# unixpickle/vq-voice-swap

Measured on AMD Instinct MI355X. Metric: audio clips/sec (whole node), unet64 50-step DDPM on 4s@16kHz waveforms, higher is better.
Workload: dtype fp16; 1 GPU; unet64 50-step DDPM (constrain, schedule t**2), 64 clips/GPU x 1 GPU of T=64000; global_batch=64, parallelism=clips sharded over 1 GPU(s), gather to rank 0

## Files before the change

### vq_voice_swap_amd/csrc/conv_ws.hip

```cpp
#include <atomic>
#include <cstddef>
#include <cstdio>
#include <cstdlib>
#include <mutex>
#include <set>
#include <string>
#include <type_traits>

#include "kernels.hpp"

namespace vqvs {

namespace {

typedef unsigned int u32x4 __attribute__((ext_vector_type(4)));
typedef int i32x4 __attribute__((ext_vector_type(4)));
typedef __attribute__((address_space(3))) void* lds_ptr;

template <typename T> struct WsOp;
template <> struct WsOp<half_t> {
  typedef f16x8 v8;
  static constexpr unsigned short one = 0x3C00;
#ifdef VQVS_F16_GELU6
  static constexpr int gq = GELU_POLY6;
// ... 15 lines not shown
__device__ __forceinline__ f32x16 ws_mfma(f16x8 a, f16x8 b, f32x16 c) { return __builtin_amdgcn_mfma_f32_32x32x16_f16(a, b, c, 0, 0, 0); }

#ifndef VQVS_WS_GELU_IL
#define VQVS_WS_GELU_IL 1
#endif
template <int Q, int N, bool IL>
__device__ __forceinline__ void ws_gelu_n(float (&v)[N]) {
  float w[N], p[N];
#define WS_G8(expr)                    \
  _Pragma("unroll") for (int i = 0; i < N; ++i) { expr; } \
  if (VQVS_WS_GELU_IL && IL) __builtin_amdgcn_sched_barrier(0);
  WS_G8(w[i] = v[i] * v[i])
  WS_G8(w[i] = __builtin_fminf(w[i], 16.0f))
  if constexpr (Q == GELU_POLY6) {
    WS_G8(p[i] = fmaf(2.81608722e-08f, w[i], -1.89188380e-06f))
    WS_G8(p[i] = fmaf(p[i], w[i], 5.41903041e-05f))
    WS_G8(p[i] = fmaf(p[i], w[i], -8.78980255e-04f))
    WS_G8(p[i] = fmaf(p[i], w[i], 9.11294959e-03f))
    WS_G8(p[i] = fmaf(p[i], w[i], -6.53883549e-02f))
    WS_G8(p[i] = fmaf(p[i], w[i], 3.98526915e-01f))
  } else {
    WS_G8(p[i] = fmaf(-1.301278171e-09f, w[i], 1.041951057e-07f))
    WS_G8(p[i] = fmaf(p[i], w[i], -3.657111166e-06f))
    WS_G8(p[i] = fmaf(p[i], w[i], 7.485478930e-05f))
    WS_G8(p[i] = fmaf(p[i], w[i], -1.006488756e-03f))
    WS_G8(p[i] = fmaf(p[i], w[i], 9.505392772e-03f))
    WS_G8(p[i] = fmaf(p[i], w[i], -6.588783436e-02f))
    WS_G8(p[i] = fmaf(p[i], w[i], 3.986733897e-01f))
  }
  WS_G8(p[i] = __builtin_amdgcn_fmed3f(fmaf(v[i], p[i], 0.5f), 0.0f, 1.0f))
  WS_G8(v[i] = v[i] * p[i])
#undef WS_G8
}

template <int Q>
__device__ __forceinline__ float ws_gelu(float v) {
  const float w = __builtin_fminf(v * v, 16.0f);
  float p;
  if constexpr (Q == GELU_POLY6) {
    p = fmaf(2.81608722e-08f, w, -1.89188380e-06f);
    p = fmaf(p, w, 5.41903041e-05f);
    p = fmaf(p, w, -8.78980255e-04f);
    p = fmaf(p, w, 9.11294959e-03f);
    p = fmaf(p, w, -6.53883549e-02f);
    p = fmaf(p, w, 3.98526915e-01f);
  } else {
    p = fmaf(-1.301278171e-09f, w, 1.041951057e-07f);
    p = fmaf(p, w, -3.657111166e-06f);
    p = fmaf(p, w, 7.485478930e-05f);
    p = fmaf(p, w, -1.006488756e-03f);
    p = fmaf(p, w, 9.505392772e-03f);
    p = fmaf(p, w, -6.588783436e-02f);
    p = fmaf(p, w, 3.986733897e-01f);
  }
  return v * __builtin_amdgcn_fmed3f(fmaf(v, p, 0.5f), 0.0f, 1.0f);
}

struct WsSeg {
  const void* src;
  const float2* ss;
  int Csrc;
  int clip_bytes;
  int c0;
  int nch;
  int ntaps;
  int dil;
  int rsz;
  int ss_lds;
  int ss_stride, ss_c0;
  int wbase, wstep;
  int lds_off;
};
struct WsGn {
  const float *part0, *part1;
  int ntiles0, ntiles1, C0, C1;
  int nsrc, Ctot, cpg, nclips;
  int tpc;
  double inv_count;
  const float *gamma, *beta, *film;
  int film_stride, film_off;
  unsigned* status;
  int guard;
};
struct WsArgs {
  WsGn gn;
  WsSeg seg[4];
  int nseg, nchunks;
  const void* w;
  const void* w_lo;
  int w_bytes;
  const float* bias;
  const void* skip;
  int skip_L, skip_rsz;
  void* out;
  float* stats;
  int Cout, Lout, TTO, ntx, nty, ntiles, ntiles_stat;
  int wres_bytes;
  int ss_bytes;
  int ss_ring;
  int rev;
  int zp;
};
static_assert(offsetof(WsArgs, gn) == 0, "gn_table reads WsGn through the kernarg segment pointer: it must stay the first member");
#define WS_SEGF(s, f) ((s) == 0 ? a.seg[0].f : ((s) == 1 ? a.seg[1].f : ((s) == 2 ? a.seg[2].f : a.seg[3].f)))

#ifndef VQVS_WS_PREP_EARLY
#define VQVS_WS_PREP_EARLY 1
#endif
constexpr int ws_lookahead(bool prep_early) { return prep_early ? 5 : 4; }
constexpr int WS_LOOKAHEAD = ws_lookahead(VQVS_WS_PREP_EARLY != 0);
constexpr int ws_ss_ring(long long spc, int lookahead) { return spc >= lookahead ? 2 : (spc >= 2 ? 4 : 8); }
constexpr int ws_ss_span(int spc, int lookahead) {
  int worst = 0;
  for (int o = 0; o < spc; ++o) {
    int clip = 0, pos = o;
    for (int i = 0; i < lookahead; ++i)
      if (++pos == spc) {
        pos = 0;
        ++clip;
      }
    worst = clip > worst ? clip : worst;
  }
  return worst;
}
constexpr bool ws_ss_ring_holds(int lookahead) {
  for (int spc = 1; spc <= 64; ++spc) {
    const int ring = ws_ss_ring(spc, lookahead);
    if ((ring & (ring - 1)) != 0 || ws_ss_span(spc, lookahead) >= ring) return false;
  }
  return true;
}
static_assert(ws_ss_ring_holds(ws_lookahead(true)) && ws_ss_ring_holds(ws_lookahead(false)),
              "the (scale, shift) ring is overwritten while a producer wave still reads it: ws_ss_ring vs. the load cursor's lookahead");
static_assert(ws_ss_ring(4, ws_lookahead(true)) == 4 && ws_ss_ring(4, ws_lookahead(false)) == 2, "ring at four steps per clip");

struct TileCo {
  int b, tx, ty;
};

#ifndef VQVS_WS_EXP
#define VQVS_WS_EXP 0
#endif

#ifdef VQVS_TIMING
__device__ unsigned long long g_ws_timing[32];
#define WS_TMARK(i)                                                \
  {                                                                \
    const unsigned long long _t = __builtin_amdgcn_s_memtime();    \
    tacc[i] += _t - tlast;                                         \
    tlast = _t;                                                    \
  }
#else
#define WS_TMARK(i)
#endif

template <typename T, int ROWS>
constexpr int ws_threads() { return sizeof(T) == 4 ? 1024 : ROWS * 4; }
template <typename T, int ROWS, int CT, bool RES, bool AVG, bool ZP = false>
__global__ __launch_bounds__((ws_threads<T, ROWS>())) void conv_ws_kernel(const WsArgs a) {
  constexpr bool X3 = sizeof(T) == 4;
  constexpr bool TALL = X3 && ROWS == 128;
  constexpr int WN = (CT == 128 && !TALL) ? 2 : 1;
  constexpr int MT = CT == 32 ? 1 : 2;
  constexpr int RW = 32 * MT;
  constexpr int NWT = ROWS / RW;
  constexpr int NWC = CT / (WN * 32);
  constexpr int NCW = NWT * NWC;
  constexpr int NPT = NCW * 64;
  constexpr int PR = ROWS * 4 / NPT;
  constexpr int HR = ROWS / 2;
  constexpr bool DB = CT == 32;
  constexpr int ES = (int)sizeof(T);
  constexpr bool L4 = AVG || (X3 && !TALL);
  static_assert(!(AVG && X3), "avg-pooled segments are not built for fp32 storage");
  static_assert(!X3 || (CT == 64 && ROWS == 256) || (CT == 128 && ROWS == 128), "fp32 storage: 256 x 64 or 128 x 128 tiles");
  static_assert(PR == 1 || PR == 2, "producer rows per chunk");
  static_assert(!TALL || !RES, "the 128 x 128 fp32 tile streams its weights (two planes of 3 x 128 x 64 B per chunk)");
  static_assert(!ZP || (!X3 && !RES && !AVG && ROWS == 256 && CT >= 64), "whole-clip tiles: 2-byte storage, streaming 256-row tiles of 64 / 128 channels");
  constexpr int ACT_BYTES = ROWS * 64;
  constexpr int W_BYTES = 3 * CT * 64;
  constexpr int ACT2 = (X3 ? 2 : 1) * ACT_BYTES, W2 = (X3 ? 2 : 1) * W_BYTES;
  constexpr int STAGE = ACT2 + W2;
  constexpr int OP = CT * 4 + 16;
  constexpr bool WPE = RES && WN == 2 && !X3;
  constexpr int ACT_STRIDE = RES ? ACT2 : STAGE;
  constexpr int WS_OFF = ACT2;
  constexpr int WS_STRIDE = STAGE;
  constexpr int O_OFF = RES ? 2 * ACT2 : 2 * STAGE;
  constexpr int O_BYTES = X3 ? 0 : (WPE ? NCW * 2048 : (ROWS / 2) * OP);
  constexpr int R_BYTES = NWT * CT * 8;
  constexpr int R_OFF = O_OFF + (DB ? 2 : 1) * O_BYTES;
  constexpr int C_OFF = R_OFF + (DB ? 2 : 1) * R_BYTES;
  constexpr int WRES_OFF = C_OFF + (RES ? 4096 : 0);
  const int SS_OFF = WRES_OFF + (RES ? (X3 ? 2 : 1) * a.wres_bytes : 0);
  constexpr int GQ = WsOp<T>::gq;
  typedef typename WsOp<T>::v8 V8;
  extern __shared__ __attribute__((aligned(16))) char smem[];

  const int tid = threadIdx.x;
  const int lane = tid & 63;
  const int wave = __builtin_amdgcn_readfirstlane(tid >> 6);
#ifdef VQVS_TIMING
  unsigned long long tacc[8] = {0, 0, 0, 0, 0, 0, 0, 0};
  unsigned long long tlast = __builtin_amdgcn_s_memtime();
  const unsigned long long t_sh0 = tlast, t_rt0 = __builtin_amdgcn_s_memrealtime();
#endif

  int tb, te;
  {
    const int nwg = (int)gridDim.x, w = (int)blockIdx.x;
    const int nx = nwg < 8 ? nwg : 8;
    const int k = w % nx, i = w / nx;
    const int nk = (nwg - k + nx - 1) / nx;
    const unsigned tot = (unsigned)a.ntiles;
    const unsigned s = tot * (unsigned)k / (unsigned)nx, e = tot * (unsigned)(k + 1) / (unsigned)nx;
    const unsigned len = e - s;
    tb = (int)(s + len * (unsigned)i / (unsigned)nk);
    te = (int)(s + len * (unsigned)(i + 1) / (unsigned)nk);
  }
  const int n = a.nchunks;
  const int Q = (te - tb) * n;
  if (Q <= 0) return;
  TileCo first;
  {
    const int ft = a.rev ? a.ntiles - 1 - tb : tb;
    const int rest = ft / a.nty;
    first.ty = ft - rest * a.nty;
    first.b = rest / a.ntx;
    first.tx = rest - first.b * a.ntx;
  }
  auto next_tile = [&](TileCo& t) {
    if (a.rev) {
      if (--t.ty < 0) {
        t.ty = a.nty - 1;
        if (--t.tx < 0) {
          t.tx = a.ntx - 1;
          --t.b;
        }
      }
    } else if (++t.ty == a.nty) {
      t.ty = 0;
      if (++t.tx == a.ntx) {
        t.tx = 0;
        ++t.b;
      }
    }
  };
  bool skipb = false;
  auto sync_lds = [&]() {
    asm volatile("s_waitcnt lgkmcnt(0)" ::: "memory");
    if (!(VQVS_WS_EXP & 32768) && !((VQVS_WS_EXP & 131072) && skipb)) __builtin_amdgcn_s_barrier();
    asm volatile("" ::: "memory");
  };

  if (wave >= NCW) {
    const int pt = tid - NPT;
    const int oct = pt & 3, r0 = pt >> 2;
    const int dst0 = r0 * 64 + ((oct ^ ((r0 >> 2) & 3)) << 4);
    struct Raw {
      u32x4 a0, a1;
      u32x4 b0, b1;
// ... 491 lines not shown
        __builtin_amdgcn_raw_buffer_store_b128(e, rs_o, v, 0, 0);
        __builtin_amdgcn_raw_buffer_store_b128(o, rs_o, v + a.Cout * 2, 0, 0);
      }
    };

    TileCo ct = first, nt_ = first;
    int cci = 0;
    struct SegW {
      int nch, ntaps, dil, wbase, wstep, lds_off;
    };
    auto fetchw = [&](int sg) -> SegW {
      const WsSeg& g = a.seg[sg];
      return SegW{g.nch, g.ntaps, g.dil, g.wbase, g.wstep, g.lds_off};
    };
    int dseg = 0, dch = 0;
    SegW dw = fetchw(0), dnx = fetchw(a.nseg > 1 ? 1 : 0);
    int d_woff = dw.wbase;
    auto wlds = [&](int par) { return dw.ntaps == 0 ? dch : (RES ? WRES_OFF + dw.lds_off + dch * dw.wstep : WS_OFF + par * WS_STRIDE); };
    if constexpr (RES) {
      const int nsg = a.nseg;
      for (int sg = 0; sg < nsg; ++sg) {
        const int np = (WS_SEGF(sg, nch) * WS_SEGF(sg, wstep)) >> 10;
        const int gb = WS_SEGF(sg, wbase), lb = WS_SEGF(sg, lds_off);
        for (int p = wave; p < np; p += NCW) {
          __builtin_amdgcn_raw_ptr_buffer_load_lds(rs_w, (lds_ptr)(smem + WRES_OFF + lb + p * 1024), 16, gb + p * 1024 + dma_lane, 0, 0, 0);
          if constexpr (X3)
            __builtin_amdgcn_raw_ptr_buffer_load_lds(rs_wl, (lds_ptr)(smem + WRES_OFF + a.wres_bytes + lb + p * 1024), 16, gb + p * 1024 + dma_lane, 0, 0, 0);
        }
      }
    }
    auto dma_advance = [&]() {
      if (++dch == dw.nch) {
        dch = 0;
        if (++dseg == a.nseg) {
          dseg = 0;
          next_tile(nt_);
        }
        dw = dnx;
        d_woff = dw.wbase;
        dnx = fetchw(dseg + 1 == a.nseg ? 0 : dseg + 1);
      } else {
        d_woff += dw.wstep;
      }
    };
    dma(dw.ntaps, d_woff, nt_, 0);
    int ntaps = dw.ntaps, d = dw.dil, wb = wlds(0);
    dma_advance();
    float bj[WN], bjn[WN];
#pragma unroll
    for (int nt = 0; nt < WN; ++nt) bjn[nt] = bj[nt] = a.bias[first.ty * CT + wc * (WN * 32) + nt * 32 + l31];
    int bias_ty = first.ty;
    const int last_b = (a.rev ? a.ntiles - te : te - 1) / (a.ntx * a.nty);
    auto reaches = [&](int c) { return a.rev ? (c >= last_b && c <= first.b) : (c >= first.b && c <= last_b); };
    if (a.gn.nsrc > 0)
      for (int i = 0; i < (a.ss_ring >> 1); ++i) {
        const int c = first.b + (a.rev ? -i : i);
        if (reaches(c)) gn_table(c);
      }
#ifdef VQVS_TIMING
    const unsigned long long t_su1 = __builtin_amdgcn_s_memtime();
#endif
    asm volatile("s_waitcnt lgkmcnt(0)" ::: "memory");
    __builtin_amdgcn_s_barrier();
#ifdef VQVS_TIMING
    const unsigned long long t_su2 = __builtin_amdgcn_s_memtime();
#endif
    constexpr int NKS = (WPE || ZP) ? 1 : 2;
    int aoff[3][NKS], aoff_d = -1;
    int aoff1[ZP ? 3 : 1];
    (void)aoff1;
    asm volatile("s_waitcnt vmcnt(0)" ::: "memory");
#ifdef VQVS_TIMING
    const unsigned long long t_su3 = __builtin_amdgcn_s_memtime();
#endif
    sync_all();
#ifdef VQVS_TIMING
    const unsigned long long t_su4 = __builtin_amdgcn_s_memtime();
#endif
    WS_TMARK(4)
    if (VQVS_WS_EXP & 1024) {
      for (int g = 0; g < Q; ++g) sync_all();
      return;
    }
    for (int g = 0; g < Q; ++g) {
      if (cci == 0) {
        if (gn_ahead != 0 && ct.b != gn_clip) {
          gn_clip = ct.b;
          if (reaches(ct.b + gn_ahead)) gn_table(ct.b + gn_ahead);
        }
        WS_TMARK(6)
        if ((n == 1 || (VQVS_WS_EXP & 256)) && pending) {
          store_tile(0, NIT);
          pending = false;
        }
        if (ct.ty != bias_ty) {
          bias_ty = ct.ty;
#pragma unroll
          for (int nt = 0; nt < WN; ++nt) bj[nt] = bjn[nt];
        }
        if (a.nty > 1) {
          TileCo nxt = ct;
          next_tile(nxt);
#pragma unroll
          for (int nt = 0; nt < WN; ++nt) bjn[nt] = a.bias[nxt.ty * CT + wc * (WN * 32) + nt * 32 + l31];
        }
#pragma unroll
        for (int nt = 0; nt < WN; ++nt)
#pragma unroll
          for (int r = 0; r < 16; ++r)
#pragma unroll
            for (int mt = 0; mt < MT; ++mt) acc[mt][nt][r] = bj[nt];
      }
      WS_TMARK(0)
      const int nx_ntaps = dw.ntaps, nx_dil = dw.dil, nx_wb = wlds((g + 1) & 1);
      if (g + 1 < Q) {
        dma(dw.ntaps, d_woff, nt_, (g + 1) & 1);
        dma_advance();
      }
      WS_TMARK(1)
      const char* const sb = smem + (g & 1) * ACT_STRIDE;
      float skv[MT][16];
      if constexpr (X3) {
        if (cci == n - 1 && a.skip != nullptr) {
          const int t0 = ct.tx * a.TTO;
          const int lastrow = t0 + min(a.TTO, a.Lout - t0);
          const int srows = a.skip_rsz == RESIZE_UP2 ? (lastrow + 1) >> 1 : (a.skip_rsz == RESIZE_AVG2 ? 2 * lastrow : lastrow);
          const __amdgpu_buffer_rsrc_t rs_s = __builtin_amdgcn_make_buffer_rsrc(
              const_cast<float*>(reinterpret_cast<const float*>(a.skip)) + (size_t)ct.b * a.skip_L * a.Cout, 0, srows * a.Cout * 4, 0x00020000);
          const int row0 = t0 + wt * RW + 4 * hh;
          const int ch4 = (ct.ty * CT + wc * (WN * 32) + l31) * 4;
#pragma unroll
          for (int mt = 0; mt < MT; ++mt)
#pragma unroll
            for (int r = 0; r < 16; ++r) {
              const int row = row0 + mt * 32 + (r & 3) + 8 * (r >> 2);
              if (a.skip_rsz == RESIZE_AVG2) {
                const float x0 = __builtin_bit_cast(float, __builtin_amdgcn_raw_buffer_load_b32(rs_s, (2 * row) * a.Cout * 4 + ch4, 0, 0));
                const float x1 = __builtin_bit_cast(float, __builtin_amdgcn_raw_buffer_load_b32(rs_s, (2 * row + 1) * a.Cout * 4 + ch4, 0, 0));
                skv[mt][r] = (x0 + x1) * 0.5f;
              } else {
                const int sr = a.skip_rsz == RESIZE_UP2 ? (row >> 1) : row;
                skv[mt][r] = __builtin_bit_cast(float, __builtin_amdgcn_raw_buffer_load_b32(rs_s, sr * a.Cout * 4 + ch4, 0, 0));
              }
            }
        }
      }
      {
        if (d != aoff_d) {
          aoff_d = d;
#pragma unroll
          for (int k = 0; k < 3; ++k) {
            if constexpr (ZP) {
              int row = wt * RW + l31 + (k - 1) * d, row1 = row + 32;
              row = (unsigned)row < 256u ? row : 255;
              row1 = (unsigned)row1 < 256u ? row1 : 255;
              aoff[k][0] = row * 64 + ((hh ^ ((row >> 2) & 3)) << 4);
              aoff1[k] = row1 * 64 + ((hh ^ ((row1 >> 2) & 3)) << 4);
            } else {
            const int row = wt * RW + l31 + k * d;
#pragma unroll
            for (int ks = 0; ks < NKS; ++ks) aoff[k][ks] = (row * 64 + ((hh ^ ((row >> 2) & 3)) << 4)) ^ (ks * 32);
            }
          }
        }
        int bad[WN][NKS];
#pragma unroll
        for (int nt = 0; nt < WN; ++nt)
#pragma unroll
          for (int ks = 0; ks < NKS; ++ks)
          bad[nt][ks] = ((ntaps != 0 ? wb + nt * (32 * 64) : ((RES ? C_OFF : WS_OFF + (g & 1) * WS_STRIDE) + (wc * WN + nt == wb ? 0 : 2048) - wc * (WN * 32 * 64))) + boff) ^ (ks * 32);
        auto tap = [&](int k) {
#pragma unroll
          for (int ks = 0; ks < 2; ++ks) {
            const int ao = NKS == 2 ? aoff[k][ks % NKS] : (aoff[k][0] ^ (ks * 32));
            const V8 a0 = *reinterpret_cast<const V8*>(sb + ao);
            V8 a1 = a0;
            if constexpr (ZP) a1 = *reinterpret_cast<const V8*>(sb + (aoff1[k] ^ (ks * 32)));
            else if constexpr (MT == 2) a1 = *reinterpret_cast<const V8*>(sb + ao + 32 * 64);
#pragma unroll
            for (int nt = 0; nt < WN; ++nt) {
              const V8 bf = *reinterpret_cast<const V8*>(smem + (NKS == 2 ? bad[nt][ks % NKS] : (bad[nt][0] ^ (ks * 32))) + k * (CT * 64));
              if constexpr (X3) {
                const V8 bl = *reinterpret_cast<const V8*>(smem + bad[nt][ks % NKS] + k * (CT * 64) + (RES ? a.wres_bytes : W_BYTES));
                const V8 a0l = *reinterpret_cast<const V8*>(sb + ACT_BYTES + ao);
                const V8 a1l = *reinterpret_cast<const V8*>(sb + ACT_BYTES + ao + 32 * 64);
                acc[0][nt] = ws_mfma(a0, bf, acc[0][nt]);
                acc[MT - 1][nt] = ws_mfma(a1, bf, acc[MT - 1][nt]);
                acc[0][nt] = ws_mfma(a0l, bf, acc[0][nt]);
                acc[MT - 1][nt] = ws_mfma(a1l, bf, acc[MT - 1][nt]);
                acc[0][nt] = ws_mfma(a0, bl, acc[0][nt]);
                acc[MT - 1][nt] = ws_mfma(a1, bl, acc[MT - 1][nt]);
              } else if (VQVS_WS_EXP & 4096) {
                asm volatile("" ::"v"(a0), "v"(a1), "v"(bf));
              } else {
                acc[0][nt] = ws_mfma(a0, bf, acc[0][nt]);
                if constexpr (MT == 2) acc[MT - 1][nt] = ws_mfma(a1, bf, acc[MT - 1][nt]);
              }
            }
          }
        };
        if (!(VQVS_WS_EXP & 16)) {
          tap(0);
          if (ntaps == 3) {
            tap(1);
            tap(2);
          }
        }
      }
      WS_TMARK(2)
      if (cci == n - 1 && (VQVS_WS_EXP & 32)) {
#pragma unroll
        for (int mt = 0; mt < MT; ++mt)
#pragma unroll
          for (int nt = 0; nt < WN; ++nt) asm volatile("" ::"v"(acc[mt][nt][0]), "v"(acc[mt][nt][15]));
        pt_ = ct;
        pbuf = obuf;
        pending = true;
      }
      if (cci == n - 1 && !(VQVS_WS_EXP & 32)) {
        int zl = 0;
        asm volatile("" : "+v"(zl));
        const int t0 = ct.tx * a.TTO;
        const int nvalid = min(a.TTO, a.Lout - t0);
        const int lim = nvalid - (wt * RW + 4 * hh) + zl;
        if (wt * RW + RW > nvalid) {
#pragma unroll
          for (int mt = 0; mt < MT; ++mt)
#pragma unroll
            for (int nt = 0; nt < WN; ++nt)
#pragma unroll
              for (int r = 0; r < 16; ++r)
                if (mt * 32 + (r & 3) + 8 * (r >> 2) >= lim) acc[mt][nt][r] = 0.f;
        }
        if constexpr (X3) {
          const int ch = ct.ty * CT + wc * (WN * 32) + l31 + zl;
          float* const outf = reinterpret_cast<float*>(a.out);
          const __amdgpu_buffer_rsrc_t rs_o = __builtin_amdgcn_make_buffer_rsrc(
              outf + (size_t)ct.b * a.Lout * a.Cout, 0, (t0 + nvalid) * a.Cout * 4, 0x00020000);
          const int row0 = t0 + wt * RW + 4 * hh;
          if (a.skip != nullptr) {
#pragma unroll
            for (int mt = 0; mt < MT; ++mt)
#pragma unroll
              for (int r = 0; r < 16; ++r) acc[mt][0][r] += skv[mt][r];
          }
          float s1 = 0.f, s2 = 0.f;
#pragma unroll
          for (int mt = 0; mt < MT; ++mt)
#pragma unroll
            for (int r = 0; r < 16; ++r) {
              const float v = acc[mt][0][r];
              s1 += v;
              s2 = fmaf(v, v, s2);
              if (!(VQVS_WS_EXP & 4))
                __builtin_amdgcn_raw_buffer_store_b32(__builtin_bit_cast(unsigned, v), rs_o, ((row0 + mt * 32 + (r & 3) + 8 * (r >> 2)) * a.Cout + ch) * 4, 0, 0);
            }
          s1 += __shfl_xor(s1, 32);
          s2 += __shfl_xor(s2, 32);
          if (hh == 0) reinterpret_cast<float2*>(smem + R_OFF)[wt * CT + wc * (WN * 32) + l31 + zl] = float2{s1, s2};
        } else if constexpr (WPE) {
          char* const priv = smem + O_OFF + wave * 2048 + zl;
          char* const wr0 = priv + (2 * hh) * 256 + l31 * 4;
          const int zlane = lane + zl;
          const int prw = zlane >> 3;
          const int rrow = (prw >> 2) * 32 + ((prw >> 1) & 1) * 4 + (prw & 1) * 2;
          const char* const rd0 = priv + prw * 256 + (zlane & 7) * 32;
          const __amdgpu_buffer_rsrc_t rs_o = __builtin_amdgcn_make_buffer_rsrc(
              outp + (size_t)ct.b * a.Lout * CT, 0, (t0 + nvalid) * (CT * 2), 0x00020000);
          const int vo0 = ((t0 + wt * 64 + rrow) * CT + wc * 64 + (zlane & 7) * 8) * 2;
          float s1[2] = {0.f, 0.f}, s2[2] = {0.f, 0.f};
#pragma unroll
          for (int j = 0; j < 4; ++j) {
#pragma unroll
            for (int mt = 0; mt < 2; ++mt)
#pragma unroll
              for (int rr = 0; rr < 2; ++rr)
#pragma unroll
                for (int nt = 0; nt < 2; ++nt) {
                  const int r = 4 * j + 2 * rr;
                  char* const o0 = wr0 + (mt * 4 + rr) * 256 + nt * 128;
                  if constexpr (WsOp<T>::one == 0x3C00) {
                    typedef _Float16 h2 __attribute__((ext_vector_type(2)));
                    const h2 ones = {(_Float16)1.0f, (_Float16)1.0f};
                    const h2 pk = {(_Float16)acc[mt][nt][r], (_Float16)acc[mt][nt][r + 1]};
                    s1[nt] = __builtin_amdgcn_fdot2(pk, ones, s1[nt], false);
                    s2[nt] = __builtin_amdgcn_fdot2(pk, pk, s2[nt], false);
                    *reinterpret_cast<h2*>(o0) = pk;
                  } else {
// ... 60 lines not shown
        }
        }
        pt_ = ct;
        pbuf = obuf;
        if constexpr (DB) obuf ^= 1;
        pending = true;
      }
      WS_TMARK(3)
      if (++cci == n) {
        cci = 0;
        next_tile(ct);
      }
      ntaps = nx_ntaps;
      d = nx_dil;
      wb = nx_wb;
      if (n > 1 && pending && cci >= 1) {
        if constexpr (!RES) asm volatile("s_waitcnt vmcnt(0)" ::: "memory");
        const int i0 = (cci - 1) * st_per, i1 = i0 + st_per;
        if (!(VQVS_WS_EXP & 4) && i0 < NIT) store_tile(i0, i1 < NIT ? i1 : NIT);
        if (i1 >= NIT) pending = false;
        asm volatile("s_waitcnt lgkmcnt(0)" ::: "memory");
        if (!(VQVS_WS_EXP & 32768) && !((VQVS_WS_EXP & 131072) && (g & 1) == 0 && g < Q - 1)) __builtin_amdgcn_s_barrier();
        asm volatile("" ::: "memory");
      } else {
        skipb = (g & 1) == 0 && g < Q - 1;
        sync_all();
        skipb = false;
      }
      WS_TMARK(4)
    }
    if (pending) store_tile(0, NIT);
#ifdef VQVS_TIMING
    WS_TMARK(5)
    if (lane == 0 && ((int)blockIdx.x & 15) == 3) {
      for (int i = 0; i < 7; ++i) atomicAdd(&g_ws_timing[8 + i], tacc[i]);
      atomicAdd(&g_ws_timing[22], t_su1 - t_sh0);
      atomicAdd(&g_ws_timing[23], t_su2 - t_su1);
      atomicAdd(&g_ws_timing[24], t_su3 - t_su2);
      atomicAdd(&g_ws_timing[25], t_su4 - t_su3);
      atomicAdd(&g_ws_timing[20], __builtin_amdgcn_s_memtime() - t_sh0);
      atomicAdd(&g_ws_timing[21], __builtin_amdgcn_s_memrealtime() - t_rt0);
      atomicAdd(&g_ws_timing[17], 1ull);
      atomicAdd(&g_ws_timing[19], (unsigned long long)(te - tb));
    }
#endif
  }
}

int ws_enabled() {
  static int v = -1;
  if (v < 0) {
    const char* e = getenv("VQVS_WS");
    v = e ? atoi(e) : 1;
  }
  return v;
}

constexpr int WS_MAX_DEV = 64;
int ws_cur_dev() {
  int dev = 0;
  if (hipGetDevice(&dev) != hipSuccess || dev < 0 || dev >= WS_MAX_DEV) return 0;
  return dev;
}
int ws_num_cus() {
  static std::atomic<int> n[WS_MAX_DEV];
  const int dev = ws_cur_dev();
  int v = n[dev].load(std::memory_order_relaxed);
  if (v == 0) {
    hipDeviceProp_t p;
    v = (hipGetDeviceProperties(&p, dev) == hipSuccess && p.multiProcessorCount > 0) ? p.multiProcessorCount : 256;
    n[dev].store(v, std::memory_order_relaxed);
  }
  return v;
}

constexpr int ws_fixed_lds(int rows, int ct, bool res, bool x3 = false) {
  const int ncw = rows / 32, nwt = ct == 32 ? rows / 32 : rows / 64, db = ct == 32 ? 2 : 1, pl = x3 ? 2 : 1;
  const int obytes = x3 ? 0 : ((res && ct == 128) ? ncw * 2048 : (rows / 2) * (ct * 4 + 16));
  return (res ? 2 * pl * rows * 64 : 2 * pl * (rows * 64 + 3 * ct * 64)) + db * obytes + db * nwt * ct * 8 + (res ? 4096 : 0);
}
constexpr int WS_LDS_MAX = 160 * 1024;
constexpr int ws_lds_cap(int rows, bool x3 = false) { return (rows == 256 || x3) ? WS_LDS_MAX : WS_LDS_MAX / 2; }

template <typename T, int ROWS, int CT, bool RES, bool AVG, bool ZP = false>
int ws_launch(const WsArgs& w, hipStream_t st) {
  constexpr bool X3 = sizeof(T) == 4;
  const int lds = ws_fixed_lds(ROWS, CT, RES, X3) + (RES ? (X3 ? 2 : 1) * w.wres_bytes : 0) + w.ss_ring * w.ss_bytes;
  static std::atomic<bool> attr_done[WS_MAX_DEV];
  const int dev = ws_cur_dev();
  if (!attr_done[dev].load(std::memory_order_acquire)) {
    VQVS_HIP(hipFuncSetAttribute(reinterpret_cast<const void*>(&conv_ws_kernel<T, ROWS, CT, RES, AVG, ZP>), hipFuncAttributeMaxDynamicSharedMemorySize, ws_lds_cap(ROWS, X3)));
    attr_done[dev].store(true, std::memory_order_release);
  }
  static const int grid_env = getenv("VQVS_WS_GRID") ? atoi(getenv("VQVS_WS_GRID")) : 0;
  constexpr int NT = ws_threads<T, ROWS>();
  const int nwg = (grid_env > 0 ? grid_env : ws_num_cus()) * (1024 / NT);
  const int grid = w.ntiles < nwg ? w.ntiles : nwg;
  static const int trace = getenv("VQVS_WS_TRACE") ? atoi(getenv("VQVS_WS_TRACE")) : 0;
  if (trace) {
    char line[320];
    snprintf(line, sizeof line, "conv_ws: prec=%s Cout=%d Lout=%d B=%d rows=%d CT=%d res=%d avg=%d zp=%d ntx=%d nty=%d nchunks=%d spc=%d ss_ring=%d la=%d ss_bytes=%d gn=%d rev=%d ntiles=%d grid=%d lds=%d",
             X3 ? "fp32" : (sizeof(T) == 2 && std::is_same<T, half_t>::value ? "fp16" : "bf16"), w.Cout, w.Lout, w.ntiles / (w.ntx * w.nty), ROWS, CT, RES ? 1 : 0,
             AVG ? 1 : 0, w.zp, w.ntx, w.nty, w.nchunks, w.ntx * w.nty * w.nchunks, w.ss_ring, WS_LOOKAHEAD, w.ss_bytes, w.gn.nsrc > 0 ? 1 : 0, w.rev, w.ntiles, grid, lds);
    static std::mutex mu;
    static std::set<std::string> seen;
    std::lock_guard<std::mutex> lk(mu);
    if (seen.insert(line).second) fprintf(stderr, "%s\n", line);
  }
  hipLaunchKernelGGL((conv_ws_kernel<T, ROWS, CT, RES, AVG, ZP>), dim3(grid), dim3(NT), lds, st, w);
  VQVS_HIP(hipGetLastError());
  return 0;
}
template <typename T, int ROWS, int CT>
int ws_launch_f(const WsArgs& w, bool res, bool avg, hipStream_t st) {
  if (avg && res) return -1;
  if (avg) return ws_launch<T, ROWS, CT, false, true>(w, st);
  return res ? ws_launch<T, ROWS, CT, true, false>(w, st) : ws_launch<T, ROWS, CT, false, false>(w, st);
}
int ws_launch_f32(const WsArgs& w, int rows, bool res, hipStream_t st) {
  if (rows == 128) return res ? -1 : ws_launch<float, 128, 128, false, false>(w, st);
  return res ? ws_launch<float, 256, 64, true, false>(w, st) : ws_launch<float, 256, 64, false, false>(w, st);
}
template <typename T>
int ws_launch_t(const WsArgs& w, int rows, int CT, bool res, bool avg, hipStream_t st) {
  if (w.zp) {
    if (rows != 256 || res || avg || CT < 64) return -1;
    return CT == 128 ? ws_launch<T, 256, 128, false, false, true>(w, st) : ws_launch<T, 256, 64, false, false, true>(w, st);
  }
  if (rows == 128) {
    if (CT == 128) return ws_launch_f<T, 128, 128>(w, res, avg, st);
    if (CT == 64) return ws_launch_f<T, 128, 64>(w, res, avg, st);
    return -1;
  }
  if (CT == 128) return ws_launch_f<T, 256, 128>(w, res, avg, st);
  if (CT == 64) return ws_launch_f<T, 256, 64>(w, res, avg, st);
  return ws_launch_f<T, 256, 32>(w, res, avg, st);
}

}

#ifdef VQVS_TIMING
int ws_timing_read(unsigned long long* out32, int reset) {
  VQVS_HIP(hipDeviceSynchronize());
  VQVS_HIP(hipMemcpyFromSymbol(out32, HIP_SYMBOL(g_ws_timing), 32 * sizeof(unsigned long long)));
  if (reset) {
    unsigned long long z[32] = {};
    VQVS_HIP(hipMemcpyToSymbol(HIP_SYMBOL(g_ws_timing), z, sizeof(z)));
  }
  return 0;
}
#endif

namespace {
struct WsPlan {
  WsArgs w;
  int CT, rows;
  bool res, avg, gn;
};
bool ws_plan(const ConvArgs& a, int B, int precision, WsPlan& plan);
}

int ws_f32_enabled() {
  static const int v = getenv("VQVS_WS_F32") ? atoi(getenv("VQVS_WS_F32")) : 1;
  return v;
}
bool ws_available(int precision) { return ws_enabled() != 0 && (precision != 0 || ws_f32_enabled() != 0); }

bool ws_fuses_gn(const ConvArgs& a, int B, int precision) {
  WsPlan plan;
  return a.gn != nullptr && ws_plan(a, B, precision, plan) && plan.gn;
}

int launch_conv_ws(const ConvArgs& a, int B, int precision, hipStream_t st) {
  WsPlan plan;
  if (!ws_plan(a, B, precision, plan)) return 0;
  if (a.gn != nullptr && !plan.gn) return 0;
  const int rc = precision == 0 ? ws_launch_f32(plan.w, plan.rows, plan.res, st)
                 : precision == 2 ? ws_launch_t<half_t>(plan.w, plan.rows, plan.CT, plan.res, plan.avg, st)
                                  : ws_launch_t<bf16_t>(plan.w, plan.rows, plan.CT, plan.res, plan.avg, st);
  return rc < 0 ? rc : 1;
}

namespace {
bool ws_plan(const ConvArgs& a, int B, int precision, WsPlan& plan) {
  const bool x3 = precision == 0;
  if (!ws_available(precision) || (x3 && (!a.ws_f32 || a.w_lo == nullptr || a.Cout % 64 != 0))) return 0;
  const int es = x3 ? 4 : 2;
  if (a.Cout % 32 != 0 || a.out_f32 || a.epi_gelu || a.nbw || (a.out_rows != 0 && a.out_rows != a.Lout)) return 0;
  auto len_ok = [&](int rsz, int Lsrc) { return rsz == RESIZE_UP2 ? Lsrc * 2 == a.Lout : (rsz == RESIZE_AVG2 ? Lsrc / 2 == a.Lout : Lsrc == a.Lout); };
  if ((long long)a.Lout * a.Cout * es >= (1LL << 31)) return 0;
  if (a.skip != nullptr && (a.skip_C != a.Cout || !len_ok(a.skip_resize, a.skip_L) || (long long)a.skip_L * a.skip_C * es >= (1LL << 29))) return 0;
  bool avg = a.skip != nullptr && a.skip_resize == RESIZE_AVG2;
  int dmax0 = 0;
  for (int s = 0; s < a.nseg; ++s)
    if (a.seg[s].ntaps == 3 && a.seg[s].dil > dmax0) dmax0 = a.seg[s].dil;
  const bool tall = x3 && a.Cout % 128 == 0 && a.tile_rows > 0 && a.tile_rows == 128 - 2 * dmax0;
  int CT = x3 ? (tall ? 128 : 64) : (a.Cout % 128 == 0 ? 128 : (a.Cout % 64 == 0 ? 64 : 32));
  static const int narrow_env = getenv("VQVS_WS_NARROW") ? atoi(getenv("VQVS_WS_NARROW")) : 1;
  if (narrow_env && !x3 && CT == 128 && a.Cout >= 256 && a.tile_rows > 0) {
    const long long rt = a.Lout <= 255 ? 1 : (a.Lout + a.tile_rows - 1) / a.tile_rows;
    if (rt * (a.Cout / 128) * B * 2 <= ws_num_cus()) CT = 64;
  }
  plan.w = WsArgs{};
  WsArgs& w = plan.w;
  int dmax = 0, n = 0;
  for (int s = 0; s < a.nseg; ++s) {
    const SegDesc& g = a.seg[s];
    if (g.C % 32 != 0 || (g.ntaps != 1 && g.ntaps != 3) || !len_ok(g.resize, g.Lsrc) || g.src2 != nullptr) return 0;
    if ((long long)g.Lsrc * g.Csrc * es >= (1LL << 29)) return 0;
    avg = avg || g.resize == RESIZE_AVG2;
    WsSeg& q = w.seg[s];
    q.src = g.src;
    q.ss = g.ss;
    q.Csrc = g.Csrc;
    q.clip_bytes = g.Lsrc * g.Csrc * es;
    q.c0 = g.c0;
    q.nch = g.C / 32;
    q.ntaps = g.ntaps;
    q.dil = g.ntaps == 3 ? g.dil : 0;
    q.rsz = g.resize;
    q.ss_stride = g.ss_stride;
    q.ss_c0 = g.ss_c0;
    q.ss_lds = w.ss_bytes;
    if (g.ss != nullptr) w.ss_bytes += g.C * 8;
    q.wbase = (int)(g.w_off * 2);
    q.wstep = g.ntaps * a.Cout * 64;
    q.lds_off = w.wres_bytes;
    w.wres_bytes += q.nch * q.wstep;
    if (q.dil > dmax) dmax = q.dil;
    n += q.nch;
  }
  w.nseg = a.nseg;
  if (a.skip != nullptr && x3) {
    w.skip = a.skip;
    w.skip_L = a.skip_L;
    w.skip_rsz = a.skip_resize;
  } else if (a.skip != nullptr) {
    WsSeg& q = w.seg[w.nseg++];
    q.src = a.skip;
    q.ss = nullptr;
    q.Csrc = a.skip_C;
    q.clip_bytes = a.skip_L * a.skip_C * 2;
    q.c0 = 0;
    q.nch = CT / 32;
    q.ntaps = 0;
    q.dil = 0;
    q.rsz = a.skip_resize;
    n += q.nch;
  }
  if (x3 && (avg || (!tall && a.tile_rows != 256 - 2 * dmax))) return 0;
  const int rows = a.tile_rows == 256 - 2 * dmax ? 256 : (a.tile_rows == 128 - 2 * dmax && CT >= 64 && a.tile_rows > 0 ? 128 : 0);
  if (rows == 0 || a.w_bytes > 0x7fffffffLL || n < (CT == 32 ? 1 : 2)) return 0;
  plan.rows = rows;
  w.nchunks = n;
  w.w = a.w_hi;
  w.w_lo = a.w_lo;
  w.w_bytes = (int)a.w_bytes;
  w.bias = a.bias;
  w.out = a.out;
  w.stats = a.stats;
  w.Cout = a.Cout;
  w.Lout = a.Lout;
  w.TTO = a.tile_rows;
  w.ntx = (a.Lout + a.tile_rows - 1) / a.tile_rows;
  w.nty = a.Cout / CT;
  static const int zp_env = getenv("VQVS_WS_ZP") ? atoi(getenv("VQVS_WS_ZP")) : 1;
  if (zp_env && !x3 && CT >= 64 && !avg && rows == 256 && a.Lout <= 255 && w.ntx > 1 && w.nty > 1) {
    w.zp = 1;
    w.TTO = 256;
    w.ntx = 1;
  }
  w.ntiles = w.ntx * w.nty * B;
  w.ntiles_stat = a.ntiles;
  static const int rev_env = getenv("VQVS_WS_REV") ? atoi(getenv("VQVS_WS_REV")) : 1;
  w.rev = rev_env ? a.rev : 0;
  if (w.ntiles <= 0) return 0;
  static const int res_env = getenv("VQVS_WS_RES") ? atoi(getenv("VQVS_WS_RES")) : 1;
  if (w.ss_bytes > 8192) return 0;
  const long long spc = (long long)w.ntx * w.nty * n;
  w.ss_ring = ws_ss_ring(spc, WS_LOOKAHEAD);
  const int ss_total = w.ss_ring * w.ss_bytes;
  if (ws_fixed_lds(rows, CT, false, x3) + ss_total > ws_lds_cap(rows, x3)) return 0;
  if (w.ntiles >= (1 << 24)) return 0;
  plan.CT = CT;
  plan.avg = avg;
  plan.res = res_env && !avg && !tall && w.nty == 1 && ws_fixed_lds(rows, CT, true, x3) + (x3 ? 2 : 1) * w.wres_bytes + ss_total <= ws_lds_cap(rows, x3);
  if (plan.res && CT == 128 && (long long)a.Lout * CT * 2 >= (1LL << 31)) return 0;
  plan.gn = false;
  static const int gn_env = getenv("VQVS_WS_GN") ? atoi(getenv("VQVS_WS_GN")) : 1;
  static const int gn_max_tiles = getenv("VQVS_WS_GN_TILES") ? atoi(getenv("VQVS_WS_GN_TILES")) : 32;
  if (a.gn != nullptr && gn_env) {
    const GnArgs& g = *a.gn;
    const int cpg = g.groups > 0 ? g.Ctot / g.groups : 0;
    bool ok = g.nsrc >= 1 && g.nsrc <= 2 && g.mr == nullptr && cpg >= 1 && cpg <= 64 && (cpg & (cpg - 1)) == 0 && g.Ctot % 64 == 0 &&
              g.src[0].C % 64 == 0 && g.Ctot * 8 == w.ss_bytes;
    int si = 0;
    for (int s = 0; s < a.nseg && ok; ++s) {
      if (a.seg[s].ss == nullptr) continue;
      ok = si < g.nsrc && a.seg[s].c0 == 0 && a.seg[s].C == g.src[si].C && a.seg[s].Csrc == g.src[si].C && g.src[si].ntiles <= gn_max_tiles;
      ++si;
    }
    ok = ok && si == g.nsrc;
    if (ok) {
      WsGn& G = w.gn;
      G.nsrc = g.nsrc;
      G.part0 = g.src[0].partials;
      G.ntiles0 = g.src[0].ntiles;
      G.C0 = g.src[0].C;
      G.part1 = g.nsrc > 1 ? g.src[1].partials : nullptr;
      G.ntiles1 = g.nsrc > 1 ? g.src[1].ntiles : 0;
      G.C1 = g.nsrc > 1 ? g.src[1].C : 0;
      G.nclips = B;
      G.Ctot = g.Ctot;
      G.cpg = cpg;
      {
        int mt = 0;
        for (int i = 0; i < g.nsrc; ++i) mt = g.src[i].ntiles > mt ? g.src[i].ntiles : mt;
        int tpc = 1;
        while (tpc < 8 && mt > 8 * tpc && cpg * 2 * tpc <= 64) tpc *= 2;
        G.tpc = tpc;
      }
      G.inv_count = g.inv_count;
      G.gamma = g.gamma;
      G.beta = g.beta;
      G.film = g.film;
      G.film_stride = g.film_stride;
      G.film_off = g.film_off;
      G.status = g.status;
      G.guard = g.guard;
      plan.gn = true;
    }
  }
  return true;
}
}

}
```

Baseline: 67.14 clips/s.

## Carry trailing 1x1 skip segment through registers instead of the LDS chunk pipeline

For resident 256x64 fp16/bf16 tiles whose last input segment is a pointwise (no-tap) skip projection, the plan strips those chunks from the LDS-staged chunk loop. Each wave instead prefetches the skip activations straight into registers with buffer loads for the next tile and applies them with extra MFMAs at the last chunk. This shortens the per-tile chunk count, shrinks the scale/shift ring and overlaps the skip loads with the main taps. The cost is a new kernel variant, more register pressure, and extra vmcnt waits at clip and GroupNorm-table boundaries.

Result: no change. 67.65 clips/s, median of 6 (+0.8%).

```diff
diff --git a/vq_voice_swap_amd/csrc/conv_ws.hip b/vq_voice_swap_amd/csrc/conv_ws.hip
--- a/vq_voice_swap_amd/csrc/conv_ws.hip
+++ b/vq_voice_swap_amd/csrc/conv_ws.hip
@@ -121,10 +121,20 @@
   unsigned* status;
   int guard;
 };
+struct WsCar {
+  const void* src;
+  int clip_bytes;
+  int row_bytes;
+  int ch_bytes;
+  int up2;
+};
+constexpr int WS_MAX_CAR = 2;
 struct WsArgs {
   WsGn gn;
   WsSeg seg[4];
   int nseg, nchunks;
+  int ncar;
+  WsCar car[WS_MAX_CAR];
   const void* w;
   const void* w_lo;
   int w_bytes;
@@ -195,7 +205,7 @@
 
 template <typename T, int ROWS>
 constexpr int ws_threads() { return sizeof(T) == 4 ? 1024 : ROWS * 4; }
-template <typename T, int ROWS, int CT, bool RES, bool AVG, bool ZP = false>
+template <typename T, int ROWS, int CT, bool RES, bool AVG, bool ZP = false, bool CAR = false>
 __global__ __launch_bounds__((ws_threads<T, ROWS>())) void conv_ws_kernel(const WsArgs a) {
   constexpr bool X3 = sizeof(T) == 4;
   constexpr bool TALL = X3 && ROWS == 128;
@@ -216,6 +226,7 @@
   static_assert(PR == 1 || PR == 2, "producer rows per chunk");
   static_assert(!TALL || !RES, "the 128 x 128 fp32 tile streams its weights (two planes of 3 x 128 x 64 B per chunk)");
   static_assert(!ZP || (!X3 && !RES && !AVG && ROWS == 256 && CT >= 64), "whole-clip tiles: 2-byte storage, streaming 256-row tiles of 64 / 128 channels");
+  static_assert(!CAR || (!X3 && RES && !AVG && !ZP && ROWS == 256 && CT == 64), "carried chunks: 2-byte storage, resident 256 x 64 tiles (the form with registers to spare)");
   constexpr int ACT_BYTES = ROWS * 64;
   constexpr int W_BYTES = 3 * CT * 64;
   constexpr int ACT2 = (X3 ? 2 : 1) * ACT_BYTES, W2 = (X3 ? 2 : 1) * W_BYTES;
@@ -873,11 +884,53 @@
       for (int g = 0; g < Q; ++g) sync_all();
       return;
     }
+    u32x4 cA[2][2] = {};
+    (void)cA;
+    auto car_load = [&](u32x4 (&buf)[2][2], int k, const TileCo& t) {
+      const WsCar& c = a.car[k];
+      const unsigned long long clip = reinterpret_cast<unsigned long long>(c.src) + (unsigned long long)(unsigned)t.b * (unsigned)c.clip_bytes;
+      i32x4 rs;
+      rs[0] = __builtin_amdgcn_readfirstlane((int)(unsigned)clip);
+      rs[1] = __builtin_amdgcn_readfirstlane((int)((unsigned)(clip >> 32) & 0xffffu));
+      rs[2] = __builtin_amdgcn_readfirstlane(c.clip_bytes);
+      rs[3] = __builtin_amdgcn_readfirstlane(0x00020000);
+      const int row = t.tx * a.TTO + wt * RW + l31;
+      const int sr0 = c.up2 ? (row >> 1) : row, sr1 = c.up2 ? ((row + 32) >> 1) : row + 32;
+      const int vo0 = sr0 * c.row_bytes + c.ch_bytes + hh * 16, vo1 = sr1 * c.row_bytes + c.ch_bytes + hh * 16;
+      asm volatile(
+          "s_nop 4\n\t"
+          "buffer_load_dwordx4 %0, %4, %6, 0 offen\n\t"
+          "buffer_load_dwordx4 %1, %4, %6, 0 offen offset:32\n\t"
+          "buffer_load_dwordx4 %2, %5, %6, 0 offen\n\t"
+          "buffer_load_dwordx4 %3, %5, %6, 0 offen offset:32"
+          : "=&v"(buf[0][0]), "=&v"(buf[0][1]), "=&v"(buf[1][0]), "=&v"(buf[1][1])
+          : "v"(vo0), "v"(vo1), "s"(rs));
+    };
+    auto car_flush = [&]() { __builtin_amdgcn_s_waitcnt(0x0F70); };
+    auto car_wait = [&]() {
+      asm volatile("s_waitcnt vmcnt(0)" : "+v"(cA[0][0]), "+v"(cA[0][1]), "+v"(cA[1][0]), "+v"(cA[1][1]));
+    };
+    auto car_mma = [&](const u32x4 (&buf)[2][2], int bb) {
+#pragma unroll
+      for (int ks = 0; ks < 2; ++ks) {
+        const V8 bf = *reinterpret_cast<const V8*>(smem + (bb ^ (ks * 32)));
+        acc[0][0] = ws_mfma(__builtin_bit_cast(V8, buf[0][ks]), bf, acc[0][0]);
+        acc[MT - 1][0] = ws_mfma(__builtin_bit_cast(V8, buf[1][ks]), bf, acc[MT - 1][0]);
+      }
+    };
+    auto car_next = [&](const TileCo& t) {
+      car_load(cA, wc, t);
+    };
+    if constexpr (CAR) {
+      car_flush();
+      car_next(first);
+    }
     for (int g = 0; g < Q; ++g) {
       if (cci == 0) {
         if (gn_ahead != 0 && ct.b != gn_clip) {
           gn_clip = ct.b;
           if (reaches(ct.b + gn_ahead)) gn_table(ct.b + gn_ahead);
+          if constexpr (CAR) car_flush();
         }
         WS_TMARK(6)
         if ((n == 1 || (VQVS_WS_EXP & 256)) && pending) {
@@ -901,6 +954,12 @@
           for (int r = 0; r < 16; ++r)
 #pragma unroll
             for (int mt = 0; mt < MT; ++mt) acc[mt][nt][r] = bj[nt];
+        if constexpr (CAR) {
+          if (pending) {
+            if (!(VQVS_WS_EXP & 4)) store_tile(0, NIT);
+            pending = false;
+          }
+        }
       }
       WS_TMARK(0)
       const int nx_ntaps = dw.ntaps, nx_dil = dw.dil, nx_wb = wlds((g + 1) & 1);
@@ -995,6 +1054,17 @@
           if (ntaps == 3) {
             tap(1);
             tap(2);
+          }
+        }
+      }
+      if constexpr (CAR) {
+        if (cci == n - 1) {
+          car_wait();
+          car_mma(cA, C_OFF + l31 * 64 + ((hh ^ ((l31 >> 2) & 3)) << 4));
+          if (g + 1 < Q) {
+            TileCo nxt = ct;
+            next_tile(nxt);
+            car_next(nxt);
           }
         }
       }
@@ -1221,14 +1291,14 @@
 constexpr int WS_LDS_MAX = 160 * 1024;
 constexpr int ws_lds_cap(int rows, bool x3 = false) { return (rows == 256 || x3) ? WS_LDS_MAX : WS_LDS_MAX / 2; }
 
-template <typename T, int ROWS, int CT, bool RES, bool AVG, bool ZP = false>
+template <typename T, int ROWS, int CT, bool RES, bool AVG, bool ZP = false, bool CAR = false>
 int ws_launch(const WsArgs& w, hipStream_t st) {
   constexpr bool X3 = sizeof(T) == 4;
   const int lds = ws_fixed_lds(ROWS, CT, RES, X3) + (RES ? (X3 ? 2 : 1) * w.wres_bytes : 0) + w.ss_ring * w.ss_bytes;
   static std::atomic<bool> attr_done[WS_MAX_DEV];
   const int dev = ws_cur_dev();
   if (!attr_done[dev].load(std::memory_order_acquire)) {
-    VQVS_HIP(hipFuncSetAttribute(reinterpret_cast<const void*>(&conv_ws_kernel<T, ROWS, CT, RES, AVG, ZP>), hipFuncAttributeMaxDynamicSharedMemorySize, ws_lds_cap(ROWS, X3)));
+    VQVS_HIP(hipFuncSetAttribute(reinterpret_cast<const void*>(&conv_ws_kernel<T, ROWS, CT, RES, AVG, ZP, CAR>), hipFuncAttributeMaxDynamicSharedMemorySize, ws_lds_cap(ROWS, X3)));
     attr_done[dev].store(true, std::memory_order_release);
   }
   static const int grid_env = getenv("VQVS_WS_GRID") ? atoi(getenv("VQVS_WS_GRID")) : 0;
@@ -1238,15 +1308,15 @@
   static const int trace = getenv("VQVS_WS_TRACE") ? atoi(getenv("VQVS_WS_TRACE")) : 0;
   if (trace) {
     char line[320];
-    snprintf(line, sizeof line, "conv_ws: prec=%s Cout=%d Lout=%d B=%d rows=%d CT=%d res=%d avg=%d zp=%d ntx=%d nty=%d nchunks=%d spc=%d ss_ring=%d la=%d ss_bytes=%d gn=%d rev=%d ntiles=%d grid=%d lds=%d",
+    snprintf(line, sizeof line, "conv_ws: prec=%s Cout=%d Lout=%d B=%d rows=%d CT=%d res=%d avg=%d zp=%d ntx=%d nty=%d nchunks=%d spc=%d ss_ring=%d la=%d ss_bytes=%d gn=%d rev=%d ntiles=%d grid=%d lds=%d carry=%d",
              X3 ? "fp32" : (sizeof(T) == 2 && std::is_same<T, half_t>::value ? "fp16" : "bf16"), w.Cout, w.Lout, w.ntiles / (w.ntx * w.nty), ROWS, CT, RES ? 1 : 0,
-             AVG ? 1 : 0, w.zp, w.ntx, w.nty, w.nchunks, w.ntx * w.nty * w.nchunks, w.ss_ring, WS_LOOKAHEAD, w.ss_bytes, w.gn.nsrc > 0 ? 1 : 0, w.rev, w.ntiles, grid, lds);
+             AVG ? 1 : 0, w.zp, w.ntx, w.nty, w.nchunks + w.ncar, w.ntx * w.nty * (w.nchunks + w.ncar), w.ss_ring, WS_LOOKAHEAD, w.ss_bytes, w.gn.nsrc > 0 ? 1 : 0, w.rev, w.ntiles, grid, lds, w.ncar);
     static std::mutex mu;
     static std::set<std::string> seen;
     std::lock_guard<std::mutex> lk(mu);
     if (seen.insert(line).second) fprintf(stderr, "%s\n", line);
   }
-  hipLaunchKernelGGL((conv_ws_kernel<T, ROWS, CT, RES, AVG, ZP>), dim3(grid), dim3(NT), lds, st, w);
+  hipLaunchKernelGGL((conv_ws_kernel<T, ROWS, CT, RES, AVG, ZP, CAR>), dim3(grid), dim3(NT), lds, st, w);
   VQVS_HIP(hipGetLastError());
   return 0;
 }
@@ -1261,7 +1331,11 @@
   return res ? ws_launch<float, 256, 64, true, false>(w, st) : ws_launch<float, 256, 64, false, false>(w, st);
 }
 template <typename T>
-int ws_launch_t(const WsArgs& w, int rows, int CT, bool res, bool avg, hipStream_t st) {
+int ws_launch_t(const WsArgs& w, int rows, int CT, bool res, bool avg, bool car, hipStream_t st) {
+  if (car) {
+    if (rows != 256 || CT != 64 || !res || avg || w.zp) return -1;
+    return ws_launch<T, 256, 64, true, false, false, true>(w, st);
+  }
   if (w.zp) {
     if (rows != 256 || res || avg || CT < 64) return -1;
     return CT == 128 ? ws_launch<T, 256, 128, false, false, true>(w, st) : ws_launch<T, 256, 64, false, false, true>(w, st);
@@ -1295,6 +1369,7 @@
   WsArgs w;
   int CT, rows;
   bool res, avg, gn;
+  bool car;
 };
 bool ws_plan(const ConvArgs& a, int B, int precision, WsPlan& plan);
 }
@@ -1315,8 +1390,8 @@
   if (!ws_plan(a, B, precision, plan)) return 0;
   if (a.gn != nullptr && !plan.gn) return 0;
   const int rc = precision == 0 ? ws_launch_f32(plan.w, plan.rows, plan.res, st)
-                 : precision == 2 ? ws_launch_t<half_t>(plan.w, plan.rows, plan.CT, plan.res, plan.avg, st)
-                                  : ws_launch_t<bf16_t>(plan.w, plan.rows, plan.CT, plan.res, plan.avg, st);
+                 : precision == 2 ? ws_launch_t<half_t>(plan.w, plan.rows, plan.CT, plan.res, plan.avg, plan.car, st)
+                                  : ws_launch_t<bf16_t>(plan.w, plan.rows, plan.CT, plan.res, plan.avg, plan.car, st);
   return rc < 0 ? rc : 1;
 }
 
@@ -1425,6 +1500,28 @@
   plan.avg = avg;
   plan.res = res_env && !avg && !tall && w.nty == 1 && ws_fixed_lds(rows, CT, true, x3) + (x3 ? 2 : 1) * w.wres_bytes + ss_total <= ws_lds_cap(rows, x3);
   if (plan.res && CT == 128 && (long long)a.Lout * CT * 2 >= (1LL << 31)) return 0;
+  static const int carry_env = getenv("VQVS_WS_CARRY") ? atoi(getenv("VQVS_WS_CARRY")) : 1;
+  plan.car = false;
+  if (carry_env && !x3 && rows == 256 && CT == 64 && plan.res && !avg && !w.zp && w.seg[w.nseg - 1].ntaps == 0) {
+    const WsSeg& q = w.seg[w.nseg - 1];
+    const int ring = ws_ss_ring((long long)w.ntx * w.nty * (n - q.nch), WS_LOOKAHEAD);
+    if ((q.rsz == RESIZE_NONE || q.rsz == RESIZE_UP2) && q.nch <= WS_MAX_CAR && n - q.nch >= 2 &&
+        ws_fixed_lds(rows, CT, true, false) + w.wres_bytes + ring * w.ss_bytes <= ws_lds_cap(rows, false)) {
+      for (int c = 0; c < q.nch; ++c) {
+        WsCar& k = w.car[w.ncar++];
+        k.src = q.src;
+        k.clip_bytes = q.clip_bytes;
+        k.row_bytes = q.Csrc * 2;
+        k.ch_bytes = (q.c0 + c * 32) * 2;
+        k.up2 = q.rsz == RESIZE_UP2 ? 1 : 0;
+      }
+      n -= q.nch;
+      --w.nseg;
+      w.nchunks = n;
+      w.ss_ring = ring;
+      plan.car = true;
+    }
+  }
   plan.gn = false;
   static const int gn_env = getenv("VQVS_WS_GN") ? atoi(getenv("VQVS_WS_GN")) : 1;
   static const int gn_max_tiles = getenv("VQVS_WS_GN_TILES") ? atoi(getenv("VQVS_WS_GN_TILES")) : 32;
```
